# wangsibovictor/fora

Hardware: AMD Instinct MI355X
Metric: SSPPR queries/sec at eps=0.5 (higher is better)
Workload: dtype u64 fixed-point 2^-62 (f64 at the boundary)

## Files before the change

### fora_amd/csrc/fora_hip.hip

```cpp
#include "fora_kernels.h"
#include "fora_team.h"
#include "fora_bwd.h"
#include "fora_sweep.h"
#include "fora_tables.h"
#include "../../include/fora_hip.h"

#include <algorithm>
#include <cmath>
#include <cstdio>
#include <cstdlib>
#include <cstring>
#include <string>
#include <unordered_map>
#include <utility>
#include <vector>

using namespace fora;

namespace {

enum EvKind { EV_PUSH_POP, EV_PUSH_EXPAND, EV_WALK_ALLOC, EV_WALK, EV_OTHER, EV_BATCH, EV_PUSH_ACCUM, EV_WALK_ACCUM, EV_ROUND_SWEEP,
              EV_PUSH_TAIL, EV_PUSH_TEAM, EV_BWD, EV_COMBINE, EV_SP_COMPACT, EV_SEED_COMBINE,
              EV_SW_COMPACT, EV_SW_SORT, EV_SW_CUT };
struct EvPair { hipEvent_t a, b; EvKind kind; };
// ... 1415 lines not shown
                               (const int32_t *)c->g.d_col.get(), (const int32_t *)w.d_ids.get(), (unsigned long long *)w.d_cut.get(), hcap);
        }
        hipLaunchKernelGGL(k_sweep_scan, dim3(nr), dim3(BLOCK), 0, c->stream, d_rd, (uint32_t)r0, w.d_cut.get(), w.d_vol.get(), hcap, (uint64_t)c->g.nnz, w.d_out.get());
        if (maxL)
            hipLaunchKernelGGL(k_sweep_scatter<false>, dim3(gx(maxL), nr), dim3(BLOCK), 0, c->stream, d_rd, (uint32_t)r0, w.d_rank.get(), n, (const int32_t *)w.d_tids.get(), tcap,
                               (const uint32_t *)nullptr, (int32_t *)nullptr, (uint64_t *)nullptr, (uint64_t *)nullptr, (uint64_t)0);
    }
    ev.end();
    HIPCHK(c, hipMemcpyAsync(w.h_out.get(), w.d_out.get(), (size_t)nb * sizeof(SweepRowOut), hipMemcpyDeviceToHost, c->stream));
    HIPCHK(c, hipStreamSynchronize(c->stream));
    const hipError_t e = hipGetLastError();
    if (e != hipSuccess) return fail(c, FORA_E_HIP, std::string("sweep: ") + hipGetErrorString(e));
    w.rank_dirty = false;
    for (int i = 0; i < nb; i++) {
        const SweepRowOut &o = w.h_out.get()[i];
        sw.rows[(size_t)at[i]] = sweep_row_of(o.len, o.best, o.cut, o.vol, o.den);
        sw.edges += o.edges;
    }
    return FORA_OK;
}

int sweep_finish(fora_ctx *c, SweepRun &sw, const int32_t *sources, int nq, int64_t *row_ptr, fora_sweep_row *rows, fora_sweep_stats *out) {
    SweepResult &w = c->swp;
    sweep_skip_dangling(sw, sources, nq);
    sw.row_ptr[(size_t)nq] = (int64_t)sw.cur;
    if (int rc = sweep_reserve(c, sw.cur, sw.cur, (uint64_t)nq, (uint64_t)nq)) return rc;
    DevBuf<int64_t> at; DevBuf<int32_t> src;
    const size_t nd = sw.dang_at.size();
    if (nd) {
        HIPCHK(c, at.alloc(nd));
        HIPCHK(c, src.alloc(nd));
        HIPCHK(c, hipMemcpyAsync(at.get(), sw.dang_at.data(), nd * 8, hipMemcpyHostToDevice, c->stream));
        HIPCHK(c, hipMemcpyAsync(src.get(), sw.dang_src.data(), nd * 4, hipMemcpyHostToDevice, c->stream));
        hipLaunchKernelGGL(k_sweep_single, dim3((unsigned)((nd + BLOCK - 1) / BLOCK)), dim3(BLOCK), 0, c->stream, (uint32_t)nd, (const int64_t *)at.get(),
                           (const int32_t *)src.get(), w.d_ids.get(), w.d_cut.get(), w.d_vol.get(), (uint64_t)w.d_ids.size());
    }
    HIPCHK(c, hipStreamSynchronize(c->stream));
    const hipError_t e = hipGetLastError();
    if (e != hipSuccess) return fail(c, FORA_E_HIP, std::string("sweep result: ") + hipGetErrorString(e));
    ev_collect(c);
    w.entries = sw.cur;
    w.valid = true;
    memcpy(row_ptr, sw.row_ptr.data(), ((size_t)nq + 1) * 8);
    if (rows && nq) memcpy(rows, sw.rows.data(), (size_t)nq * sizeof(fora_sweep_row));
    if (out) {
        memset(out, 0, sizeof(*out));
        out->entries = sw.entries_len; out->max_row = sw.max_row; out->thr_fix = sw.thr; out->edges = sw.edges;
        out->batches = sw.batches; out->global_rows = sw.global_rows;
        out->compact_ms = c->tm.sw_compact_ms; out->sort_ms = c->tm.sw_sort_ms; out->cut_ms = c->tm.sw_cut_ms;
    }
    return FORA_OK;
}

void launch_walks(fora_ctx *c, const Dev &d, int nq, bool with_idx, uint32_t round, int nzh) {
    const WsPlan &p = c->ws.plan;
    const dim3 wg(walk_grid_x(c, nq), nq);
    const dim3 wgs(p.binned ? p.sub : 1u, nq);
    EvSpan ev(c, EV_WALK);
    if (with_idx) {
        if (!p.binned) hipLaunchKernelGGL(k_walk_idx<1>, wg, dim3(BLOCK), 0, c->stream, d);
        else if (!d.wide) hipLaunchKernelGGL(k_walk_idx<MAX_BINS>, wgs, dim3(BLOCK), 0, c->stream, d);
        else
            for (int lo = 0; lo < p.nbins; lo += p.pbins) {
                Dev dp = d;
                dp.bin_lo = lo;
                dp.bin_cnt = std::min(p.pbins, p.nbins - lo);
                const dim3 wgi = (dp.slot_major & 4u) ? dim3(wgs.y, wgs.x) : wgs;
                if (p.pbins > MAX_BINS_WIDE) hipLaunchKernelGGL(k_walk_idx<MAX_BINS_HUGE>, wgi, dim3(BIN_THREADS_HUGE), 0, c->stream, dp);
                else hipLaunchKernelGGL(k_walk_idx<MAX_BINS_WIDE>, wgi, dim3(BIN_THREADS_WIDE), 0, c->stream, dp);
                { const unsigned gx = acc_grid(c, dp, nq); hipLaunchKernelGGL((k_accum<true, true>), (dp.slot_major & 2u) ? dim3(nq, gx) : dim3(gx, nq), dim3(ACC_THREADS_WIDE), 0, c->stream, dp, 0); }
            }
    }
    const bool dg = p.binned && !d.wide && d.dg.colp && c->opt_.walk_dg != 0;
    const bool xl = dg && c->opt_.walk_dg != 1 && d.dg.invb;
    if (xl && with_idx) {
        ev.begin(EV_WALK_ACCUM);
        hipLaunchKernelGGL((k_accum<true, false>), dim3(p.nbins, nq), dim3(ACC_THREADS), 0, c->stream, d, 0);
        ev.begin(EV_WALK);
    }
    Dev dw = d;
    if (xl) { dw.nbins = (int32_t)d.dg.nbx; dw.acc_xl = d.dg.invb; }
    if (dg) {
        const size_t lds = (xl ? (size_t)((d.dg.H + 1) & ~1u) * 8 : 0) + (size_t)4 * d.dg.nrec * 4 + (((size_t)d.dg.nblk + 3) & ~(size_t)3);
#define FORA_DG_LAUNCH(NZH, B32, XLF) hipLaunchKernelGGL((k_walk_dg<NZH, B32, XLF>), wgs, dim3(DG_THREADS), lds, c->stream, dw, round)
        const int sel = (nzh ? 4 : 0) | (d.dg.bits32 ? 2 : 0) | (xl ? 1 : 0);
        switch (sel) {
        case 0: FORA_DG_LAUNCH(false, false, false); break;
        case 1: FORA_DG_LAUNCH(false, false, true); break;
        case 2: FORA_DG_LAUNCH(false, true, false); break;
        case 3: FORA_DG_LAUNCH(false, true, true); break;
        case 4: FORA_DG_LAUNCH(true, false, false); break;
        case 5: FORA_DG_LAUNCH(true, false, true); break;
        case 6: FORA_DG_LAUNCH(true, true, false); break;
        default: FORA_DG_LAUNCH(true, true, true); break;
        }
#undef FORA_DG_LAUNCH
    } else
        hipLaunchKernelGGL(k_walk_online<WALK_TO_PPR>, p.binned && !d.wide ? wgs : wg, dim3(BLOCK), 0, c->stream, d, round, nzh, (int32_t *)nullptr);
    ev.end();
    if (p.binned && !d.wide) {
        ev.begin(EV_WALK_ACCUM);
        hipLaunchKernelGGL((k_accum<true, false>), dim3(dw.nbins, nq), dim3(ACC_THREADS), 0, c->stream, dw, 0);
    }
}

static hipError_t ensure_active(Workspace &w) { return w.d_active.ensure((size_t)w.B); }
int push_balanced(fora_ctx *c, const int32_t *sources, int nq, bool with_idx) {
    HIPCHK(c, ensure_active(c->ws));
    const uint32_t chunks = slab_grid_x(c, std::min(nq, c->ws.B));
    Dev d = make_dev(c, nq, with_idx);
    EvSpan ev(c, EV_OTHER);
    hipLaunchKernelGGL(k_init_batch, dim3((nq + BLOCK - 1) / BLOCK), dim3(BLOCK), 0, c->stream, d, 1);
    ev.end();
    std::vector<uint8_t> active((size_t)nq, 1);
    std::vector<uint64_t> rsum_fix((size_t)nq, FIX_ONE), pops((size_t)nq, 0), relax((size_t)nq, 0);
    c->bal.h_rmax_used.assign((size_t)nq, c->par.rmax);
    c->bal.h_rounds.assign((size_t)nq, 1);
    for (int i = 0; i < nq; i++)
        if (is_dangling(c, sources[i])) active[i] = 0;
    for (int i = 0; i < nq; i++) if (active[i]) c->bal.h_rounds[i] = 0;
    double rmax = c->par.rmax * c->bal.start;
    for (int round = 0;; round++) {
        bool any = false;
        for (int i = 0; i < nq; i++) {
            if (!active[i]) continue;
            const double t = (!with_idx || rmax >= c->par.rmax) ? c->bal.t_walk : c->bal.t_idx;
            const double est = c->par.omega * std::ldexp((double)rsum_fix[i], -62) * (1 - c->par.alpha) * t;
            const double used = (double)pops[i] * c->bal.c_pop + (double)relax[i] * c->bal.c_edge;
            if (!(est > used)) active[i] = 0;
            else { any = true; c->bal.h_rmax_used[i] = rmax; c->bal.h_rounds[i] = round + 1; }
        }
        if (!any) break;
        if (round >= 64) return fail(c, FORA_E_OVERFLOW, "--balanced: rmax halved 64 times");
        HIPCHK(c, hipMemcpyAsync(c->ws.d_active.get(), active.data(), (size_t)nq, hipMemcpyHostToDevice, c->stream));
        if (round) {
            HIPCHK(c, c->ws.d_counters.zero(c->stream));
            int rc = reset_binned_counters(c);
            if (rc) return rc;
        }
        Dev dr = make_dev(c, nq, with_idx, rmax, c->par.omega);
        ev.begin(EV_OTHER);
        hipLaunchKernelGGL(k_topk_frontier, dim3(chunks, nq), dim3(BLOCK), 0, c->stream, dr, (const uint8_t *)c->ws.d_active.get());
        ev.end();
        int rc = run_push_levels(c, dr, nullptr, 0, true);
        if (rc) return rc;
        HIPCHK(c, hipMemcpy(c->h_qs.data(), c->ws.d_qs.get(), (size_t)nq * sizeof(QState), hipMemcpyDeviceToHost));
        for (int i = 0; i < nq; i++) {
            rsum_fix[i] = FIX_ONE - c->h_qs[i].reserved;
            pops[i] = c->h_qs[i].pops;
// ... 645 lines not shown
    if (!(alpha > 0 && alpha < 1) || !(rmax > 0) || !(omega >= 0)) return fail(c, FORA_E_ARG, "bad params");
    c->par.alpha = alpha; c->par.rmax = rmax; c->par.omega = omega; c->par.opt = opt ? 1 : 0; c->par.seed = seed;
    c->par.have = true;
    return FORA_OK;
}

int fora_hip_get_params(fora_ctx *c, double *rmax, double *omega) {
    if (!c || !c->par.have) return FORA_E_ARG;
    if (rmax) *rmax = c->par.rmax;
    if (omega) *omega = c->par.omega;
    return FORA_OK;
}

int fora_hip_set_batch(fora_ctx *c, int batch) {
    if (!c || batch < 0) return FORA_E_ARG;
    if (batch != c->batch_req) { (void)hipSetDevice(c->device); free_workspace(c); }
    c->batch_req = batch;
    return FORA_OK;
}
int fora_hip_get_batch(fora_ctx *c) { return c ? c->ws.B : FORA_E_ARG; }

int fora_hip_set_option(fora_ctx *c, const char *name, int64_t value) {
    if (!c || !name) return FORA_E_ARG;
    if (!strcmp(name, "reset")) {
        (void)hipSetDevice(c->device);
        free_workspace(c);
        c->opt_ = tunables_from_env();
        c->team_run.suspend = 0;
        apply_options(c);
        return FORA_OK;
    }
    if (!TEST_PATHS && schedule_option(name) && value != (strcmp(name, "rounds") ? (strcmp(name, "round_div") ? 0 : 4) : 1))
        return fail(c, FORA_E_ARG, std::string("option ") + name + ": the schedule experiments are not compiled into this library (build with -DFORA_TEST_PATHS=1: libfora_hip_test.so)");
    for (const auto &o : OPTIONS)
        if (!strcmp(name, o.name)) {
            if (c->opt_.*(o.field) == value) return FORA_OK;
            c->opt_.*(o.field) = value;
            if (o.layout) { (void)hipSetDevice(c->device); free_workspace(c); }
            apply_options(c);
            return FORA_OK;
        }
    return fail(c, FORA_E_ARG, std::string("unknown option ") + name);
}

int fora_hip_get_option(fora_ctx *c, const char *name, int64_t *value) {
    if (!name || !value) return FORA_E_ARG;
    if (!strcmp(name, "test_paths")) { *value = TEST_PATHS ? 1 : 0; return FORA_OK; }
    if (!strcmp(name, "diag_build")) { *value = FORA_DIAG_BUILD; return FORA_OK; }
    if (!c) return FORA_E_ARG;
    if (!strcmp(name, "bucket_retries")) { *value = (int64_t)c->retry.retries; return FORA_OK; }
    if (!strcmp(name, "team_fallbacks")) { *value = (int64_t)c->team_run.fallbacks; return FORA_OK; }
    if (!strcmp(name, "team_suspended")) { *value = c->team_run.suspend; return FORA_OK; }
    if (!strcmp(name, "team_members")) { *value = c->g.team.T; return FORA_OK; }
    if (!strcmp(name, "team_cooperative")) { *value = c->team_run.coop_ok && !c->team_run.coop_failed ? 1 : 0; return FORA_OK; }
    for (const auto &o : OPTIONS)
        if (!strcmp(name, o.name)) { *value = c->opt_.*(o.field); return FORA_OK; }
    return fail(c, FORA_E_ARG, std::string("unknown option ") + name);
}

int fora_hip_set_balanced(fora_ctx *c, int on, double start_scale, double c_pop, double c_edge, double t_walk, double t_idx) {
    if (!c) return FORA_E_ARG;
    const Balanced def;
    c->bal.on = on != 0;
    c->bal.start = start_scale > 0 ? start_scale : def.start;
    c->bal.c_pop = c_pop > 0 ? c_pop : def.c_pop;
    c->bal.c_edge = c_edge > 0 ? c_edge : def.c_edge;
    c->bal.t_walk = t_walk > 0 ? t_walk : def.t_walk;
    c->bal.t_idx = t_idx > 0 ? t_idx : def.t_idx;
    return FORA_OK;
}

static uint64_t host_index_sizes(const fora_ctx *c, uint64_t *off, uint64_t *cnt) {
    uint64_t total = 0;
    for (int32_t v = 0; v < c->g.n; v++) {
        const size_t deg = (size_t)(c->g.h_row_ptr[v + 1] - c->g.h_row_ptr[v]);
        unsigned long num_rw;
        if (c->par.opt) num_rw = (unsigned long)ceil(deg * c->par.rmax * (1 - c->par.alpha) * c->par.omega);
        else num_rw = (unsigned long)ceil(deg * c->par.rmax * c->par.omega);
        if (off) off[v] = total;
        if (cnt) cnt[v] = num_rw;
        total += num_rw;
    }
    return total;
}

int fora_hip_index_sizes(fora_ctx *c, uint64_t *total, uint64_t *off, uint64_t *cnt) {
    if (!c || !c->g.n || !c->par.have) return fail(c, FORA_E_ARG, "set_graph and set_params first");
    const uint64_t t = host_index_sizes(c, off, cnt);
    if (total) *total = t;
    return FORA_OK;
}

int fora_hip_build_index(fora_ctx *c) {
    if (!c || !c->g.n || !c->par.have) return fail(c, FORA_E_ARG, "set_graph and set_params first");
    HIPCHK(c, hipSetDevice(c->device));
    std::vector<uint64_t> off((size_t)c->g.n), cnt((size_t)c->g.n);
    const uint64_t total = host_index_sizes(c, off.data(), cnt.data());
    free_index(c);
    Index ix;
    HIPCHK(c, ix.d_rw_idx.alloc(std::max<uint64_t>(1, total)));
    HIPCHK(c, ix.d_idx_off.alloc((size_t)c->g.n));
    HIPCHK(c, ix.d_idx_cnt.alloc((size_t)c->g.n));
    HIPCHK(c, hipMemcpy(ix.d_idx_off.get(), off.data(), (size_t)c->g.n * 8, hipMemcpyHostToDevice));
    HIPCHK(c, hipMemcpy(ix.d_idx_cnt.get(), cnt.data(), (size_t)c->g.n * 8, hipMemcpyHostToDevice));
    ix.len = total;
    c->retry.div = 1;
// ... 1106 lines not shown
```

### fora_amd/csrc/fora_kernels.h

```cpp
#pragma once
#include <hip/hip_runtime.h>
#include <stdint.h>
#include <type_traits>
#include "fora_consts.h"
#include "fora_diag.h"

namespace fora {

constexpr int BLOCK = 256;
constexpr uint32_t PUSH_SEG = 256;
constexpr uint32_t WALK_SEG = 1024;
#ifndef FORA_TEST_PATHS
#define FORA_TEST_PATHS 0
#endif
constexpr bool TEST_PATHS = FORA_TEST_PATHS != 0;
constexpr uint64_t FIX_ONE = 1ull << 62;
constexpr int MAX_LEVELS = 1 << 15;
#ifndef FORA_ACC_THREADS
#define FORA_ACC_THREADS 512
#endif
constexpr int ACC_THREADS = FORA_ACC_THREADS;
#ifndef FORA_ACC_THREADS_WIDE
#define FORA_ACC_THREADS_WIDE 1024
#endif
// ... 1981 lines not shown
                    WalkItem w = {};
                    w.j0 = (uint64_t)k * WALK_SEG;
                    const uint64_t left = num - w.j0;
                    w.cnt = left < WALK_SEG ? (uint32_t)left : WALK_SEG;
                    w.idx_pos = ioff + w.j0;
                    w.v = v;
                    d.wit[sb + off + k] = wit_pack(w);
                }
            }
        }
    }
}

enum { WALK_TO_PPR = 0, WALK_TO_INDEX = 1 };

__device__ __forceinline__ int32_t walk_one(const Dev &d, uint32_t start, uint64_t j, uint32_t stream,
                                            uint32_t round, int nzh, uint32_t &steps) {
    int64_t beg; uint64_t deg;
    node_row(d, start, beg, deg);
    if (deg == 0) return (int32_t)start;
    uint32_t cur = start;
    uint32_t w[4];
    for (uint32_t t = 0;; t++) {
        if ((t & 1u) == 0)
            philox4x32_10(start, (uint32_t)j,
                          (uint32_t)((j >> 32) & 0xFFFFu) | ((round & 0xFFu) << 16) | (((t >> 1) & 0xFFu) << 24),
                          stream ^ ((t >> 9) * 0x9E3779B9u), d.seed_lo, d.seed_hi, w);
        const uint32_t ws = (t & 1u) ? w[2] : w[0], wm = (t & 1u) ? w[3] : w[1];
        if (!(nzh && t == 0) && ws < d.alpha32) return (int32_t)cur;
        if (t) node_row(d, cur, beg, deg);
        if (deg > 0)
            cur = (uint32_t)d.col[beg + (int64_t)(((uint64_t)wm * deg) >> 32)];
        else
            cur = start;
        steps++;
    }
}

#ifndef FORA_STAGE
#define FORA_STAGE 320
#endif
#ifndef FORA_WALK_WPE
#define FORA_WALK_WPE 6
#endif
constexpr int STAGE = FORA_STAGE;
struct WaveStage {
    uint64_t *pk;
    uint32_t *bcnt;
    uint32_t *bbase;
    uint32_t *fill;
    uint32_t count;
    const uint32_t *xl;
};
template <int ST, bool XLD = false>
__device__ __forceinline__ void stage_flush(const Dev &d, int q, WaveStage &st) {
    const int lane = threadIdx.x & 63;
    const uint64_t slab = (uint64_t)q * d.n;
    const uint64_t bk0 = SubBuckets::first_of(d.pbins, d.sub, d.bk_cap, q, blockIdx.x), bstride = SubBuckets::stride_of(d.sub, d.bk_cap);
    st.bcnt[lane] = 0;
    st.bcnt[lane + 64] = 0;
    __builtin_amdgcn_wave_barrier();
    constexpr uint64_t NONE = ~0ull;
    uint32_t rk[ST / 64];
    uint64_t wv[ST / 64];
#pragma unroll
    for (int k = 0; k < ST / 64; k++) {
        const uint32_t m = k * 64 + lane;
        wv[k] = NONE;
        if (m < st.count) {
            wv[k] = st.pk[m];
            if (XLD) {
                const uint32_t lo = (uint32_t)wv[k], u = lo & ((1u << WPACK_SHIFT) - 1), blk = u >> 6;
                const uint32_t qd = __umulhi(blk, d.dg.nbx_magic);
                const uint32_t dest = ((blk - qd * d.dg.nbx) << BIN_SHIFT) | (qd << 6) | (u & 63u);
                wv[k] = (wv[k] & 0xFFFFFFFF00000000ull) | ((lo & ~((1u << WPACK_SHIFT) - 1)) | dest);
            }
            rk[k] = atomicAdd(&st.bcnt[((uint32_t)wv[k] & ((1u << WPACK_SHIFT) - 1)) >> BIN_SHIFT], 1u);
        }
    }
    __builtin_amdgcn_wave_barrier();
    {
        const uint32_t c0 = lane < d.nbins ? st.bcnt[lane] : 0, c1 = lane + 64 < d.nbins ? st.bcnt[lane + 64] : 0;
        uint32_t t0, t1;
        const uint32_t o0 = wave_excl_scan(c0, t0), o1 = wave_excl_scan(c1, t1);
        if (c0) st.bbase[lane] = atomicAdd(&st.fill[lane], c0);
        if (c1) st.bbase[lane + 64] = atomicAdd(&st.fill[lane + 64], c1);
        st.bcnt[lane] = o0;
        st.bcnt[lane + 64] = t0 + o1;
    }
    __builtin_amdgcn_wave_barrier();
#pragma unroll
    for (int k = 0; k < ST / 64; k++)
        if (wv[k] != NONE) st.pk[st.bcnt[((uint32_t)wv[k] & ((1u << WPACK_SHIFT) - 1)) >> BIN_SHIFT] + rk[k]] = wv[k];
    __builtin_amdgcn_wave_barrier();
#pragma unroll
    for (int k = 0; k < ST / 64; k++) {
        const uint32_t m = k * 64 + lane;
        if (m < st.count) {
            const uint64_t pk = st.pk[m];
            const uint32_t dd = (uint32_t)pk & ((1u << WPACK_SHIFT) - 1);
            const uint32_t b = dd >> BIN_SHIFT;
            const uint32_t pos = st.bbase[b] + (m - st.bcnt[b]);
            if (pos < d.bk_cap) __builtin_nontemporal_store(pk, &d.bk_inc[bk0 + (uint64_t)b * bstride + pos]);
            else atomicAdd((unsigned long long *)&d.ppr[slab + (st.xl ? st.xl[dd] : dd)], (unsigned long long)(pk >> WPACK_SHIFT));
        }
    }
    __builtin_amdgcn_wave_barrier();
    st.count = 0;
}
template <int ST, bool XLD = false, bool CHECKW = true>
__device__ __forceinline__ void stage_emit(const Dev &d, int q, WaveStage &st, bool has, uint32_t dest, uint64_t w) {
    if (CHECKW && has && w >= WPACK_MAXW) {
        atomicAdd((unsigned long long *)&d.ppr[(uint64_t)q * d.n + (st.xl ? st.xl[dest] : dest)], (unsigned long long)w);
        has = false;
    }
    const unsigned long long mask = __ballot(has);
    if (!mask) return;
    if (has) {
        const uint32_t pos = st.count + sp_mbcnt(mask);
        st.pk[pos] = (uint64_t)dest | (w << WPACK_SHIFT);
    }
    st.count += (uint32_t)__popcll(mask);
    if (st.count > ST - 64) stage_flush<ST, XLD>(d, q, st);
}
#define WAVE_STAGE_DECL_N(st, NWAVES, ST)                                                           \
    __shared__ uint64_t st##_pk[NWAVES][ST];                                                        \
    __shared__ uint32_t st##_bcnt[NWAVES][MAX_BINS], st##_bbase[NWAVES][MAX_BINS];                 \
    __shared__ uint32_t st##_fill[MAX_BINS];                                                        \
    WaveStage st;                                                                                   \
    st.pk = st##_pk[threadIdx.x >> 6];                                                              \
    st.bcnt = st##_bcnt[threadIdx.x >> 6]; st.bbase = st##_bbase[threadIdx.x >> 6];                 \
    st.fill = st##_fill; st.count = 0; st.xl = nullptr;
#define WAVE_STAGE_DECL(st) WAVE_STAGE_DECL_N(st, BLOCK / 64, STAGE)

template <int NB>
__global__ void __launch_bounds__(BinThreads<NB>::value) k_walk_idx(Dev d) {
    constexpr int NT = BinThreads<NB>::value;
    constexpr int EPT = NB > MAX_BINS ? FORA_IDX_EPT_WIDE : BIN_EPT;
    constexpr uint32_t CHUNK = NT * EPT;
    constexpr uint32_t PAD = NB > MAX_BINS ? FORA_RUN_PAD_WIDE : 1;
    constexpr bool BINNED = NB > 1;
    constexpr bool WIDE = NB > MAX_BINS;
    constexpr int BS = WIDE ? BIN_SHIFT_WIDE : BIN_SHIFT;
    constexpr uint32_t BSZ = 1u << BS;
    constexpr int IB = NT == 256 ? 8 : NT == 512 ? 9 : 10;
    constexpr int DB = WIDE ? BS : WPACK_SHIFT;
    static_assert(DB + IB + 1 <= 32, "stage word: destination | item | carries-one-more-unit");
    __shared__ uint64_t s_j0[NT], s_pos[NT], s_incr[NT], s_rem[NT];
    __shared__ uint32_t s_pref[NT + 1], s_w[NT / 64];
    __shared__ uint32_t s_cnt[NB], s_lofs[NB + 1], s_fill[NB];
    __shared__ uint32_t s_msg[BINNED ? CHUNK : 1];
    __shared__ uint16_t s_bin[BINNED ? CHUNK : 1];
    const bool slot_major = NB > MAX_BINS && (d.slot_major & 4u);
    const int q = slot_major ? blockIdx.x : blockIdx.y;
    const uint32_t bx = slot_major ? blockIdx.y : blockIdx.x, gx = slot_major ? gridDim.y : gridDim.x;
    const uint32_t nitems = (uint32_t)min((uint64_t)d.wit_count[q * CSTRIDE], d.wit_cap);
    if (!nitems || *d.err) return;
    const WalkItemP *items = d.wit + (uint64_t)q * d.wit_cap;
    const uint64_t slab = (uint64_t)q * d.n;
    const uint32_t bin_lo = (uint32_t)d.bin_lo;
    const BinExchange<NB, NT, PAD> ex{s_cnt, s_lofs, s_fill, s_w, SubBuckets(d.bk_count, d.pbins, d.sub, d.bk_cap, q, bx), (uint32_t)d.bin_cnt};
    if (BINNED) ex.load_fills();
    constexpr uint32_t GRAN = FORA_TILE_GRAN_WALK;
    const uint32_t ntiles = (nitems + NT - 1) / NT;
    const uint32_t seg_len = ntiles * GRAN;
    for (uint32_t tile = bx; tile < ntiles; tile += gx) {
        const uint32_t i = tile_pos<GRAN>(threadIdx.x, tile, seg_len);
        uint32_t cnt = 0;
        if (i < nitems) {
            const WalkItem w = wit_load(&items[i]);
            s_j0[threadIdx.x] = w.j0; s_pos[threadIdx.x] = w.idx_pos;
            s_incr[threadIdx.x] = w.incr; s_rem[threadIdx.x] = w.rem;
            cnt = w.idx_n;
        }
        uint32_t total;
        const uint32_t pre = block_excl_scan_n<NT>(cnt, s_w, total);
        s_pref[threadIdx.x] = pre;
        if (threadIdx.x == 0) s_pref[NT] = total;
        __syncthreads();
        for (uint32_t cb = 0; cb < total; cb += CHUNK) {
            uint32_t dest[EPT], rank[EPT], li[EPT];
            const uint32_t e0 = cb + threadIdx.x * EPT;
            uint32_t lo = e0 < total ? pref_find<NT>(s_pref, e0) : 0;
#pragma unroll
// ... 134 lines not shown
                        if (deg0 == 0) done = (int32_t)start;
                        else active = true;
                    }
                    const uint32_t want = (uint32_t)__popcll(idle);
                    wptr += want < avail ? want : avail;
                    while (wptr < wend && s_pref[cur_item + 1] <= wptr) cur_item++;
                }
                if (active)
                    philox4x32_10(start, (uint32_t)wj,
                                  (uint32_t)((wj >> 32) & 0xFFFFu) | ((round & 0xFFu) << 16) | (((t >> 1) & 0xFFu) << 24),
                                  stream ^ ((t >> 9) * 0x9E3779B9u), d.seed_lo, d.seed_hi, rw);
            }
            if (active) {
                const uint32_t ws = (it & 1u) ? rw[2] : rw[0], wm = (it & 1u) ? rw[3] : rw[1];
                if (!(nzh && t == 0) && ws < d.alpha32) {
                    done = (int32_t)cur;
                    active = false;
                } else {
                    if (t) cur = walk_move(d, cur, start, wm);
                    else if (d.rp32) cur = colp_at(d, (uint64_t)beg0 + (((uint64_t)wm * deg0) >> 32));
                    else cur = (uint32_t)d.col[beg0 + (int64_t)(((uint64_t)wm * deg0) >> 32)];
                    t++;
                    steps++;
                }
            }
            if (staged) {
                stage_emit<STAGE>(d, q, st, done >= 0, (uint32_t)done, wgt);
            } else if (done >= 0) {
                if (MODE == WALK_TO_INDEX) idx_out[opos] = done;
                else atomicAdd((unsigned long long *)&d.ppr[slab + (uint32_t)done], (unsigned long long)wgt);
            }
        }
        __syncthreads();
    }
    if (staged && st.count) stage_flush<STAGE>(d, q, st);
    if (staged) {
        __syncthreads();
        for (uint32_t i = threadIdx.x; i < (uint32_t)d.nbins; i += BLOCK) bkc[(uint64_t)i * d.sub] = st.fill[i];
    }
    const uint64_t ws = wave_sum((uint64_t)steps);
    __syncthreads();
    if ((threadIdx.x & 63) == 0) s_w[threadIdx.x >> 6] = (uint32_t)ws;
    __syncthreads();
    if (threadIdx.x == 0) {
        const unsigned long long bs = (unsigned long long)s_w[0] + s_w[1] + s_w[2] + s_w[3];
        if (bs) atomicAdd(d.tot_steps, bs);
    }
}

#ifndef FORA_DG_THREADS
#define FORA_DG_THREADS 512
#endif
#ifndef FORA_DG_STAGE
#define FORA_DG_STAGE 256
#endif
#ifndef FORA_DG_WPE
#define FORA_DG_WPE 6
#endif
constexpr int DG_THREADS = FORA_DG_THREADS;
constexpr int DG_STAGE = FORA_DG_STAGE;
#ifndef FORA_DG_TILE
#define FORA_DG_TILE 256
#endif
constexpr int DG_TILE = FORA_DG_TILE;
typedef uint32_t __attribute__((aligned(1))) u32_unaligned;
template <bool BITS32>
__device__ __forceinline__ uint32_t dg_colp_at(const WalkDG &g, uint32_t e) {
    if (BITS32) {
        const uint32_t at = g.bits * e;
        const uint32_t w = *(const u32_unaligned *)((const char *)g.colp + (at >> 3));
        return (w >> (at & 7)) & ((1u << g.bits) - 1u);
    }
    uint32_t word, sh;
    if (BITS32) { const uint32_t at = g.bits * e; word = at >> 5; sh = at & 31; }
    else { const uint64_t at = (uint64_t)g.bits * e; word = (uint32_t)(at >> 5); sh = (uint32_t)at & 31; }
    const U32Pair cw = *(const U32Pair *)(g.colp + word);
    const uint64_t both = ((uint64_t)cw.b << 32) | cw.a;
    return (uint32_t)(both >> sh) & ((1u << g.bits) - 1u);
}
template <bool NZH, bool BITS32, bool XL>
__global__ void __launch_bounds__(DG_THREADS) __attribute__((amdgpu_waves_per_eu(FORA_DG_WPE, 8))) k_walk_dg(Dev d, uint32_t round) {
    constexpr int NW = DG_THREADS / 64;
    extern __shared__ __attribute__((aligned(16))) uint64_t dg_lds64[];
    constexpr int WT = DG_TILE / NW;
    static_assert(WT >= 1 && WT <= 64, "a lane loads one item of its wave's tile");
    struct __attribute__((aligned(16))) TileItem { uint64_t jb, rem, incr; uint32_t v, vp; };
    static_assert(sizeof(TileItem) == 32, "two uint4");
    __shared__ TileItem w_item[NW][WT];
    __shared__ uint32_t w_pref[NW][WT + 1], s_w[NW];
    __shared__ unsigned long long w_self[XL ? NW : 1][XL ? WT : 1];
    __shared__ uint32_t s_ticket;
    const int q = blockIdx.y;
    const uint32_t nitems = (uint32_t)min((uint64_t)d.wit_count[q * CSTRIDE], d.wit_cap);
    if (!nitems || *d.err) return;
    const WalkDG &g = d.dg;
    const uint32_t H = g.H, ts = g.ts;
    unsigned long long *s_hub = (unsigned long long *)dg_lds64;
    uint32_t *dg_lds = (uint32_t *)(dg_lds64 + (XL ? ((H + 1) & ~1u) : 0));
    uint4 *s_rec = (uint4 *)dg_lds;
    const uint32_t ncls = g.nrec - H;
    const uint8_t *s_T = (const uint8_t *)(dg_lds + 4 * g.nrec);
    for (uint32_t i = threadIdx.x; i < g.nrec; i += DG_THREADS) s_rec[i < H ? ncls + i : i - H] = make_uint4(g.rec[i], g.rec[g.nrec + i], g.rec[2 * g.nrec + i], 0u);
    for (uint32_t i = threadIdx.x; i < (g.nblk + 3) / 4; i += DG_THREADS) dg_lds[4 * g.nrec + i] = ((const uint32_t *)g.T)[i];
    if (XL) for (uint32_t i = threadIdx.x; i < H; i += DG_THREADS) s_hub[i] = 0;
    const WalkItemP *items = d.wit + (uint64_t)q * d.wit_cap;
    const uint64_t slab = (uint64_t)q * d.n;
    const uint32_t stream = (uint32_t)d.src[q];
    const int lane = threadIdx.x & 63, wid = __builtin_amdgcn_readfirstlane((int)(threadIdx.x >> 6));
    uint32_t steps = 0;
    WAVE_STAGE_DECL_N(st, NW, DG_STAGE)
    if (XL) st.xl = g.invb;
    uint32_t *bkc = d.bk_count + (uint64_t)q * d.pbins * d.sub + blockIdx.x;
    for (uint32_t i = threadIdx.x; i < (uint32_t)MAX_BINS; i += DG_THREADS) st.fill[i] = i < (uint32_t)d.nbins ? bkc[(uint64_t)i * d.sub] : 0;
    if (threadIdx.x == 0) s_ticket = 0;
    __syncthreads();
    auto move = [&](uint32_t cur, uint32_t startp, uint32_t wm) -> uint32_t {
        uint32_t r = ncls + cur;
        if (cur >= H) r = s_T[(cur - H) >> ts];
        const uint4 rc = s_rec[r];
        const uint32_t dg = rc.y;
        const uint32_t e = rc.z + (cur - rc.x) * dg + __umulhi(wm, dg);
        const uint32_t nx = dg_colp_at<BITS32>(g, e);
        return dg ? nx : startp;
    };
    bool pend = false;
    uint32_t pend_node = 0;
    uint64_t pend_w = 0;
    unsigned long long *s_self = w_self[XL ? wid : 0];
    TileItem *s_item = w_item[wid];
    uint32_t *s_pref = w_pref[wid];
    if (XL && lane < WT) s_self[lane] = 0;
    uint32_t gen = 0, tag = 0;
    auto flush_self = [&]() {
        if (!XL) return;
        const unsigned long long sv = lane < WT ? s_self[lane] : 0ull;
        const uint32_t dn = lane < WT ? s_item[lane].vp : 0u;
        if (lane < WT && sv) s_self[lane] = 0;
        if (sv && dn < H) atomicAdd(&s_hub[dn], sv);
        bool has = sv != 0 && dn >= H;
        if (has && sv >= WPACK_MAXW) {
            atomicAdd((unsigned long long *)&d.ppr[slab + g.inv[dn]], sv);
            has = false;
        }
        stage_emit<DG_STAGE, true, false>(d, q, st, has, dn - H, (uint64_t)sv);
    };
    const uint32_t ntiles = (nitems + WT - 1) / WT;
    const uint32_t tstride = gridDim.x * NW;
    bool more = true;
    auto take_tile = [&]() -> uint32_t {
        uint32_t k = 0;
        if (lane == 0) k = atomicAdd(&s_ticket, 1u);
        return dg_ticket_tile(blockIdx.x, (uint32_t)NW, tstride, (uint32_t)__builtin_amdgcn_readfirstlane((int)k));
    };
    uint32_t wptr = 0, wend = 0;
    uint32_t cur_item = 0;
    bool big = false;
    auto advance = [&]() {
        while (wptr < wend && (uint32_t)__builtin_amdgcn_readfirstlane((int)s_pref[cur_item + 1]) <= wptr) cur_item++;
    };
    bool active = false;
    uint32_t cur = 0, start = 0, startp = 0, c1 = 0, c2 = 0, c3 = 0;
    const uint32_t c2_round = (round & 0xFFu) << 16;
    uint64_t wgt = 0;
    for (;;) {
        bool fin = false;
        const unsigned long long idle = __ballot(!active);
        if (idle && wptr == wend) {
            while (wptr == wend && more) {
                const uint32_t tile = take_tile();
                if (tile >= ntiles) { more = false; break; }
                if (gen) flush_self();
                gen++;
                const uint32_t i = tile * WT + lane;
                const bool have = lane < WT && i < nitems;
                WalkItem w = {};
                if (have) {
                    const uint64_t *wp = (const uint64_t *)&items[i];
                    const uint64_t x0 = NT_LOAD(wp), x1 = NT_LOAD(wp + 1), x3 = NT_LOAD(wp + 3);
                    w = wit_unpack(x0, x1, 0, x3);
                }
                const uint32_t cnt = have ? w.cnt - w.idx_n : 0u;
                uint32_t total;
                const uint32_t pre = wave_excl_scan(cnt, total);
                if (have) {
                    TileItem it;
                    it.jb = w.j0 + w.idx_n - pre;
                    it.rem = w.rem; it.incr = w.incr;
                    it.v = w.v; it.vp = g.perm[w.v];
                    s_item[lane] = it;
                }
                if (__ballot(have && w.incr + 1 >= WPACK_MAXW)) big = true;
                if (lane < WT) s_pref[lane] = pre;
                if (lane == 0) s_pref[WT] = total;
                __builtin_amdgcn_fence(__ATOMIC_RELEASE, "wavefront");
                __builtin_amdgcn_wave_barrier();
                wptr = 0; wend = total; cur_item = 0;
                advance();
            }
        }
        const uint32_t avail = wend - wptr;
        if (!avail && idle == ~0ull) break;
        if (avail && idle) {
            const uint32_t rank = sp_mbcnt(idle);
            if (!active && rank < avail) {
                const uint32_t e = wptr + rank;
                uint32_t item = cur_item;
                while (s_pref[item + 1] <= e) item++;
                const uint4 ia = ((const uint4 *)&s_item[item])[0], ib = ((const uint4 *)&s_item[item])[1];
                const uint64_t wj = (((uint64_t)ia.y << 32) | ia.x) + e;
                const uint64_t rem = ((uint64_t)ia.w << 32) | ia.z;
                wgt = (((uint64_t)ib.y << 32) | ib.x) + (wj < rem ? 1 : 0);
                start = ib.z;
                startp = ib.w;
                c1 = (uint32_t)wj;
                c2 = ((uint32_t)(wj >> 32) & 0xFFFFu) | c2_round;
                c3 = stream;
                cur = startp;
                tag = (gen << 6) | item;
                fin = startp >= g.zero_first;
                active = !fin;
            }
            const uint32_t want = (uint32_t)__popcll(idle);
            wptr += want < avail ? want : avail;
            advance();
            __builtin_amdgcn_wave_barrier();
        }
        if (active) {
            uint32_t rw[4];
            philox4x32_10(start, c1, c2, c3, d.seed_lo, d.seed_hi, rw);
            const uint32_t later = (c2 >> 24) | (c3 ^ stream);
            c2 += 1u << 24;
            if (__ballot(c2 < (1u << 24))) {
                asm volatile("" ::: "memory");
                if (c2 < (1u << 24)) c3 = stream ^ ((c3 ^ stream) + 0x9E3779B9u);
            }
            if (!(NZH && later == 0) && rw[0] < d.alpha32) {
                fin = true;
            } else {
                cur = move(diag::dg_from(cur, later), startp, rw[1]);
                steps++;
                if (rw[2] < d.alpha32) {
                    fin = true;
                } else {
                    cur = move(diag::dg_from(cur, 1u), startp, rw[3]);
                    steps++;
                }
            }
            active = !fin;
        }
        if (XL) {
            const bool self = fin && cur == startp && tag >= (gen << 6);
            if (self) atomicAdd(&s_self[tag & 63u], (unsigned long long)wgt);
            const bool away = fin && !self;
            if (away && cur < H) atomicAdd(&s_hub[cur], (unsigned long long)wgt);
            const bool over = big && wgt >= WPACK_MAXW;
            if (away && cur >= H && over) atomicAdd((unsigned long long *)&d.ppr[slab + g.inv[cur]], (unsigned long long)wgt);
            stage_emit<DG_STAGE, true, false>(d, q, st, away && cur >= H && !over, cur - H, wgt);
        } else {
            stage_emit<DG_STAGE>(d, q, st, pend, pend_node, pend_w);
            pend = fin;
            if (pend) { pend_node = g.inv[cur]; pend_w = wgt; }
        }
    }
    if (!XL) stage_emit<DG_STAGE>(d, q, st, pend, pend_node, pend_w);
    if (gen) flush_self();
    if (st.count) stage_flush<DG_STAGE, XL>(d, q, st);
    __syncthreads();
    for (uint32_t i = threadIdx.x; i < (uint32_t)d.nbins; i += DG_THREADS) bkc[(uint64_t)i * d.sub] = st.fill[i];
    if (XL) for (uint32_t i = threadIdx.x; i < H; i += DG_THREADS) {
        const unsigned long long hv = s_hub[i];
        if (hv) atomicAdd((unsigned long long *)&d.ppr[slab + g.inv[i]], hv);
    }
    const uint64_t ws = wave_sum((uint64_t)steps);
    if (lane == 0) s_w[wid] = (uint32_t)ws;
    __syncthreads();
    if (threadIdx.x == 0) {
        unsigned long long bs = 0;
#pragma unroll
        for (int w = 0; w < NW; w++) bs += s_w[w];
        if (bs) atomicAdd(d.tot_steps, bs);
    }
}

__global__ void __launch_bounds__(BLOCK) k_ppr_sum(Dev d) {
    const int q = blockIdx.y;
    const uint64_t slab = (uint64_t)q * d.n;
    uint64_t acc = 0;
    const uint64_t step = (uint64_t)gridDim.x * BLOCK;
    for (uint64_t v0 = (uint64_t)blockIdx.x * BLOCK + threadIdx.x; v0 < (uint64_t)d.n; v0 += step * SLAB_UNROLL) {
        uint64_t x[SLAB_UNROLL];
        slab_load(x, d.ppr, slab, v0, step, (uint64_t)d.n);
#pragma unroll
        for (int u = 0; u < SLAB_UNROLL; u++) acc += x[u];
    }
    acc = wave_sum(acc);
    if ((threadIdx.x & 63) == 0 && acc) atomicAdd(&d.qs[q].ppr_sum, (unsigned long long)acc);
}

__global__ void __launch_bounds__(BLOCK) k_walk_counts_f64(int32_t n, const double *residue, double rsum,
                                                           double omega, double alpha, int opt,
                                                           uint64_t *num_s_rw, uint64_t *n_rw) {
    double check_rsum = rsum;
    if (opt) check_rsum *= (1 - alpha);
    const uint64_t N = check_rsum == 0.0 ? 0 : (uint64_t)(omega * check_rsum);
    const int v = blockIdx.x * BLOCK + threadIdx.x;
    if (v == 0) *n_rw = N;
    if (v >= n) return;
    double r = residue[v];
    uint64_t num = 0;
    if (r > 0 && check_rsum != 0.0) {
        if (opt) r = r * (1 - alpha);
        num = walk_count(r, check_rsum, N);
    }
    num_s_rw[v] = num;
}

__global__ void __launch_bounds__(BLOCK) k_walks_raw(Dev d, uint32_t stream, uint32_t round, int nzh,
                                                     const int32_t *starts, const uint64_t *js, int64_t count,
                                                     int32_t *dests) {
// ... 285 lines not shown
```

### fora_amd/csrc/fora_tables.h

```cpp
#pragma once
#include "fora_consts.h"

#include <algorithm>
#include <cstddef>
#include <vector>

namespace fora {


inline std::vector<uint32_t> in_degrees(size_t n, const int32_t *col, size_t nnz) {
    std::vector<uint32_t> indeg(n, 0);
    for (size_t e = 0; e < nnz; e++) indeg[(size_t)col[e]]++;
    return indeg;
}
inline std::vector<uint32_t> top_by_indegree(const std::vector<uint32_t> &indeg, size_t H) {
    std::vector<uint32_t> order(indeg.size());
    for (size_t v = 0; v < order.size(); v++) order[v] = (uint32_t)v;
    H = std::min(H, order.size());
    std::partial_sort(order.begin(), order.begin() + (ptrdiff_t)H, order.end(),
                      [&](uint32_t a, uint32_t b) { return indeg[a] != indeg[b] ? indeg[a] > indeg[b] : a < b; });
    order.resize(H);
    return order;
}
template <class F> std::vector<uint32_t> pack_bits(uint64_t count, uint32_t bits, F value_of) {
    std::vector<uint32_t> pk((size_t)((count * bits + 31) / 32) + 2, 0);
    for (uint64_t e = 0; e < count; e++) {
        const uint64_t at = e * bits;
        const uint64_t x = (uint64_t)(uint32_t)value_of(e) << (at & 31);
        pk[at >> 5] |= (uint32_t)x;
        pk[(at >> 5) + 1] |= (uint32_t)(x >> 32);
    }
    return pk;
}


struct RowBasics {
    bool ok = true;
    std::vector<uint64_t> rowinfo;
    std::vector<uint32_t> deg;
    int64_t n_dangling = 0;
};
inline RowBasics make_row_basics(int32_t n, const int64_t *row_ptr) {
    RowBasics r;
    r.rowinfo.resize((size_t)n);
    r.deg.resize((size_t)n);
    for (int32_t v = 0; v < n; v++) {
        const uint64_t dg = (uint64_t)(row_ptr[v + 1] - row_ptr[v]);
        r.n_dangling += dg == 0;
        if (dg > 0xFFFFFFFFull) { r.ok = false; return r; }
        r.deg[(size_t)v] = (uint32_t)dg;
        r.rowinfo[(size_t)v] = ((uint64_t)row_ptr[v] << 24) | std::min<uint64_t>(dg, DEG_SAT);
    }
    return r;
}


struct CompactWalk {
    uint32_t bits = 0;
    std::vector<uint32_t> rp32, colp;
};
inline CompactWalk make_compact_walk(int32_t n, const int64_t *row_ptr, const int32_t *col) {
    CompactWalk w;
    w.bits = 1;
    while ((1ull << w.bits) < (uint64_t)n) w.bits++;
    if (w.bits > 31) w.bits = 31;
    w.rp32.resize((size_t)n + 1);
    for (int32_t v = 0; v <= n; v++) w.rp32[(size_t)v] = (uint32_t)row_ptr[v];
    w.colp = pack_bits((uint64_t)row_ptr[n], w.bits, [&](uint64_t e) { return col[e]; });
    return w;
}


constexpr size_t WALK_DG_LDS_CAP = 28 * 1024;
struct DgTables {
    bool have = false;
    uint32_t H = 0, nrec = 0, ts = 0, bits = 0, zero_first = 0, bits32 = 0;
    uint32_t np = 0;
    std::vector<uint32_t> perm, inv, rec, colp;
    std::vector<uint8_t> T;
    uint32_t nbx = 0, nbx_magic = 0;
    std::vector<uint32_t> invb;
};
inline DgTables make_walk_dg(int32_t n, const int64_t *row_ptr, const int32_t *col, int64_t dg_hubs) {
    DgTables t;
    const uint64_t nnz = (uint64_t)row_ptr[n];
    std::vector<uint32_t> order((size_t)n);
    for (int32_t v = 0; v < n; v++) order[(size_t)v] = (uint32_t)v;
    auto degree = [&](uint32_t v) { return (uint32_t)(row_ptr[v + 1] - row_ptr[v]); };
    std::stable_sort(order.begin(), order.end(), [&](uint32_t a, uint32_t b) { return degree(a) > degree(b); });
    uint32_t H = 0, K = 0;
    for (uint32_t h : {256u, 512u, 1024u, 2048u, 4096u}) {
        if (dg_hubs > 0 && (int64_t)h < dg_hubs) continue;
        const uint32_t hh = std::min<uint32_t>(h, (uint32_t)n);
        uint32_t k = 0;
        for (size_t i = hh; i < (size_t)n; i++) if (i == hh || degree(order[i]) != degree(order[i - 1])) k++;
        if (k <= 255) { H = hh; K = k; break; }
    }
    if (H == 0 && !(n <= 256)) return DgTables{};
    if (n <= 256) { H = (uint32_t)n; K = 0; }
    uint32_t ts = 6;
    while ((((uint64_t)n + 256ull * (1ull << ts)) >> ts) > 8192) ts++;
    const uint32_t blk = 1u << ts;
    const uint32_t nrec = H + K;
    t.rec.assign((size_t)3 * nrec, 0);
    t.perm.resize((size_t)n);
    uint32_t *first = t.rec.data(), *rdeg = t.rec.data() + nrec, *base = t.rec.data() + 2 * (size_t)nrec;
    uint64_t edge = 0;
    uint32_t id = 0, zero_first = 0xFFFFFFFFu;
    for (uint32_t i = 0; i < H; i++) {
        const uint32_t v = order[i];
        t.perm[v] = id; first[i] = id; rdeg[i] = degree(v); base[i] = (uint32_t)edge;
        if (rdeg[i] == 0 && zero_first == 0xFFFFFFFFu) zero_first = id;
        edge += rdeg[i]; id++;
    }
    uint32_t k = 0;
    for (size_t i = H; i < (size_t)n;) {
        size_t j = i;
        const uint32_t dg = degree(order[i]);
        while (j < (size_t)n && degree(order[j]) == dg) j++;
        const uint32_t r = H + k;
        first[r] = id; rdeg[r] = dg; base[r] = (uint32_t)edge;
        if (dg == 0 && zero_first == 0xFFFFFFFFu) zero_first = id;
        for (size_t u = i; u < j; u++) t.perm[order[u]] = id + (uint32_t)(u - i);
        const uint32_t cnt = (uint32_t)(j - i), padded = (cnt + blk - 1) / blk * blk;
        for (uint32_t b = 0; b < padded / blk; b++) t.T.push_back((uint8_t)k);
        edge += (uint64_t)cnt * dg;
// ... 185 lines not shown
```

Measured before the change: 7058.

## Shrink walk_dg LDS footprint: drop bbase array, 16-bit prefixes, retune stage/tile

The degree-grouped walk kernel now uses a staging variant that folds each bin's global base minus its local offset into the per-wave bcnt array, so the separate bbase shared array is no longer needed. Tile prefix sums are stored as 16-bit values, guarded by a static_assert. The stage size goes from 256 to 384 and the tile size from 256 to 128. A host-side query option reports the kernel's workgroups per CU, and the kernel selection and LDS size computation are moved into helper functions. The aim is to trade LDS between staging capacity and occupancy, and a larger stage risks lowering occupancy.

```diff
diff --git a/fora_amd/csrc/fora_hip.hip b/fora_amd/csrc/fora_hip.hip
--- a/fora_amd/csrc/fora_hip.hip
+++ b/fora_amd/csrc/fora_hip.hip
@@ -1491,6 +1491,21 @@
     return FORA_OK;
 }
 
+typedef void (*WalkDgKernel)(Dev, uint32_t);
+static WalkDgKernel walk_dg_kernel(bool nzh, bool bits32, bool xl) {
+    switch ((nzh ? 4 : 0) | (bits32 ? 2 : 0) | (xl ? 1 : 0)) {
+    case 0: return k_walk_dg<false, false, false>;
+    case 1: return k_walk_dg<false, false, true>;
+    case 2: return k_walk_dg<false, true, false>;
+    case 3: return k_walk_dg<false, true, true>;
+    case 4: return k_walk_dg<true, false, false>;
+    case 5: return k_walk_dg<true, false, true>;
+    case 6: return k_walk_dg<true, true, false>;
+    default: return k_walk_dg<true, true, true>;
+    }
+}
+static size_t walk_dg_lds(const WalkDG &g, bool xl) { return walk_dg_lds_bytes(g.H, g.nrec, g.nblk, xl); }
+
 void launch_walks(fora_ctx *c, const Dev &d, int nq, bool with_idx, uint32_t round, int nzh) {
     const WsPlan &p = c->ws.plan;
     const dim3 wg(walk_grid_x(c, nq), nq);
@@ -1520,20 +1535,7 @@
     Dev dw = d;
     if (xl) { dw.nbins = (int32_t)d.dg.nbx; dw.acc_xl = d.dg.invb; }
     if (dg) {
-        const size_t lds = (xl ? (size_t)((d.dg.H + 1) & ~1u) * 8 : 0) + (size_t)4 * d.dg.nrec * 4 + (((size_t)d.dg.nblk + 3) & ~(size_t)3);
-#define FORA_DG_LAUNCH(NZH, B32, XLF) hipLaunchKernelGGL((k_walk_dg<NZH, B32, XLF>), wgs, dim3(DG_THREADS), lds, c->stream, dw, round)
-        const int sel = (nzh ? 4 : 0) | (d.dg.bits32 ? 2 : 0) | (xl ? 1 : 0);
-        switch (sel) {
-        case 0: FORA_DG_LAUNCH(false, false, false); break;
-        case 1: FORA_DG_LAUNCH(false, false, true); break;
-        case 2: FORA_DG_LAUNCH(false, true, false); break;
-        case 3: FORA_DG_LAUNCH(false, true, true); break;
-        case 4: FORA_DG_LAUNCH(true, false, false); break;
-        case 5: FORA_DG_LAUNCH(true, false, true); break;
-        case 6: FORA_DG_LAUNCH(true, true, false); break;
-        default: FORA_DG_LAUNCH(true, true, true); break;
-        }
-#undef FORA_DG_LAUNCH
+        hipLaunchKernelGGL(walk_dg_kernel(nzh != 0, d.dg.bits32 != 0, xl), wgs, dim3(DG_THREADS), walk_dg_lds(d.dg, xl), c->stream, dw, round);
     } else
         hipLaunchKernelGGL(k_walk_online<WALK_TO_PPR>, p.binned && !d.wide ? wgs : wg, dim3(BLOCK), 0, c->stream, d, round, nzh, (int32_t *)nullptr);
     ev.end();
@@ -2285,6 +2287,18 @@
     if (!strcmp(name, "team_fallbacks")) { *value = (int64_t)c->team_run.fallbacks; return FORA_OK; }
     if (!strcmp(name, "team_suspended")) { *value = c->team_run.suspend; return FORA_OK; }
     if (!strcmp(name, "team_members")) { *value = c->g.team.T; return FORA_OK; }
+    if (!strcmp(name, "walk_dg_wgs_per_cu")) {
+        const WalkDG &g = c->g.walk.dg;
+        int wgs = 0;
+        if (g.colp) {
+            const bool xl = c->opt_.walk_dg != 1 && g.invb;
+            (void)hipSetDevice(c->device);
+            if (hipOccupancyMaxActiveBlocksPerMultiprocessor(&wgs, (const void *)walk_dg_kernel(false, g.bits32 != 0, xl), DG_THREADS, walk_dg_lds(g, xl)) != hipSuccess)
+                return fail(c, FORA_E_HIP, "hipOccupancyMaxActiveBlocksPerMultiprocessor(k_walk_dg)");
+        }
+        *value = wgs;
+        return FORA_OK;
+    }
     if (!strcmp(name, "team_cooperative")) { *value = c->team_run.coop_ok && !c->team_run.coop_failed ? 1 : 0; return FORA_OK; }
     for (const auto &o : OPTIONS)
         if (!strcmp(name, o.name)) { *value = c->opt_.*(o.field); return FORA_OK; }
diff --git a/fora_amd/csrc/fora_kernels.h b/fora_amd/csrc/fora_kernels.h
--- a/fora_amd/csrc/fora_kernels.h
+++ b/fora_amd/csrc/fora_kernels.h
@@ -2057,7 +2057,7 @@
     uint32_t count;
     const uint32_t *xl;
 };
-template <int ST, bool XLD = false>
+template <int ST, bool XLD = false, bool ONE = false>
 __device__ __forceinline__ void stage_flush(const Dev &d, int q, WaveStage &st) {
     const int lane = threadIdx.x & 63;
     const uint64_t slab = (uint64_t)q * d.n;
@@ -2068,6 +2068,7 @@
     constexpr uint64_t NONE = ~0ull;
     uint32_t rk[ST / 64];
     uint64_t wv[ST / 64];
+    uint32_t dl0 = 0, dl1 = 0;
 #pragma unroll
     for (int k = 0; k < ST / 64; k++) {
         const uint32_t m = k * 64 + lane;
@@ -2088,8 +2089,13 @@
         const uint32_t c0 = lane < d.nbins ? st.bcnt[lane] : 0, c1 = lane + 64 < d.nbins ? st.bcnt[lane + 64] : 0;
         uint32_t t0, t1;
         const uint32_t o0 = wave_excl_scan(c0, t0), o1 = wave_excl_scan(c1, t1);
-        if (c0) st.bbase[lane] = atomicAdd(&st.fill[lane], c0);
-        if (c1) st.bbase[lane + 64] = atomicAdd(&st.fill[lane + 64], c1);
+        if (ONE) {
+            if (c0) dl0 = atomicAdd(&st.fill[lane], c0) - o0;
+            if (c1) dl1 = atomicAdd(&st.fill[lane + 64], c1) - (t0 + o1);
+        } else {
+            if (c0) st.bbase[lane] = atomicAdd(&st.fill[lane], c0);
+            if (c1) st.bbase[lane + 64] = atomicAdd(&st.fill[lane + 64], c1);
+        }
         st.bcnt[lane] = o0;
         st.bcnt[lane + 64] = t0 + o1;
     }
@@ -2098,6 +2104,11 @@
     for (int k = 0; k < ST / 64; k++)
         if (wv[k] != NONE) st.pk[st.bcnt[((uint32_t)wv[k] & ((1u << WPACK_SHIFT) - 1)) >> BIN_SHIFT] + rk[k]] = wv[k];
     __builtin_amdgcn_wave_barrier();
+    if (ONE) {
+        st.bcnt[lane] = dl0;
+        st.bcnt[lane + 64] = dl1;
+        __builtin_amdgcn_wave_barrier();
+    }
 #pragma unroll
     for (int k = 0; k < ST / 64; k++) {
         const uint32_t m = k * 64 + lane;
@@ -2105,7 +2116,7 @@
             const uint64_t pk = st.pk[m];
             const uint32_t dd = (uint32_t)pk & ((1u << WPACK_SHIFT) - 1);
             const uint32_t b = dd >> BIN_SHIFT;
-            const uint32_t pos = st.bbase[b] + (m - st.bcnt[b]);
+            const uint32_t pos = ONE ? st.bcnt[b] + m : st.bbase[b] + (m - st.bcnt[b]);
             if (pos < d.bk_cap) __builtin_nontemporal_store(pk, &d.bk_inc[bk0 + (uint64_t)b * bstride + pos]);
             else atomicAdd((unsigned long long *)&d.ppr[slab + (st.xl ? st.xl[dd] : dd)], (unsigned long long)(pk >> WPACK_SHIFT));
         }
@@ -2113,7 +2124,7 @@
     __builtin_amdgcn_wave_barrier();
     st.count = 0;
 }
-template <int ST, bool XLD = false, bool CHECKW = true>
+template <int ST, bool XLD = false, bool CHECKW = true, bool ONE = false>
 __device__ __forceinline__ void stage_emit(const Dev &d, int q, WaveStage &st, bool has, uint32_t dest, uint64_t w) {
     if (CHECKW && has && w >= WPACK_MAXW) {
         atomicAdd((unsigned long long *)&d.ppr[(uint64_t)q * d.n + (st.xl ? st.xl[dest] : dest)], (unsigned long long)w);
@@ -2126,7 +2137,7 @@
         st.pk[pos] = (uint64_t)dest | (w << WPACK_SHIFT);
     }
     st.count += (uint32_t)__popcll(mask);
-    if (st.count > ST - 64) stage_flush<ST, XLD>(d, q, st);
+    if (st.count > ST - 64) stage_flush<ST, XLD, ONE>(d, q, st);
 }
 #define WAVE_STAGE_DECL_N(st, NWAVES, ST)                                                           \
     __shared__ uint64_t st##_pk[NWAVES][ST];                                                        \
@@ -2135,6 +2146,14 @@
     WaveStage st;                                                                                   \
     st.pk = st##_pk[threadIdx.x >> 6];                                                              \
     st.bcnt = st##_bcnt[threadIdx.x >> 6]; st.bbase = st##_bbase[threadIdx.x >> 6];                 \
+    st.fill = st##_fill; st.count = 0; st.xl = nullptr;
+#define WAVE_STAGE_DECL_ONE(st, NWAVES, ST)                                                         \
+    __shared__ uint64_t st##_pk[NWAVES][ST];                                                        \
+    __shared__ uint32_t st##_bcnt[NWAVES][MAX_BINS];                                                \
+    __shared__ uint32_t st##_fill[MAX_BINS];                                                        \
+    WaveStage st;                                                                                   \
+    st.pk = st##_pk[threadIdx.x >> 6];                                                              \
+    st.bcnt = st##_bcnt[threadIdx.x >> 6]; st.bbase = nullptr;                                      \
     st.fill = st##_fill; st.count = 0; st.xl = nullptr;
 #define WAVE_STAGE_DECL(st) WAVE_STAGE_DECL_N(st, BLOCK / 64, STAGE)
 
@@ -2375,7 +2394,7 @@
 #define FORA_DG_THREADS 512
 #endif
 #ifndef FORA_DG_STAGE
-#define FORA_DG_STAGE 256
+#define FORA_DG_STAGE 384
 #endif
 #ifndef FORA_DG_WPE
 #define FORA_DG_WPE 6
@@ -2383,7 +2402,7 @@
 constexpr int DG_THREADS = FORA_DG_THREADS;
 constexpr int DG_STAGE = FORA_DG_STAGE;
 #ifndef FORA_DG_TILE
-#define FORA_DG_TILE 256
+#define FORA_DG_TILE 128
 #endif
 constexpr int DG_TILE = FORA_DG_TILE;
 typedef uint32_t __attribute__((aligned(1))) u32_unaligned;
@@ -2410,7 +2429,9 @@
     struct __attribute__((aligned(16))) TileItem { uint64_t jb, rem, incr; uint32_t v, vp; };
     static_assert(sizeof(TileItem) == 32, "two uint4");
     __shared__ TileItem w_item[NW][WT];
-    __shared__ uint32_t w_pref[NW][WT + 1], s_w[NW];
+    static_assert((uint64_t)WT * WALK_SEG <= 0xFFFFu, "a tile's walk count fits the 16-bit prefix sums");
+    __shared__ uint16_t w_pref[NW][WT + 1];
+    __shared__ uint32_t s_w[NW];
     __shared__ unsigned long long w_self[XL ? NW : 1][XL ? WT : 1];
     __shared__ uint32_t s_ticket;
     const int q = blockIdx.y;
@@ -2431,7 +2452,7 @@
     const uint32_t stream = (uint32_t)d.src[q];
     const int lane = threadIdx.x & 63, wid = __builtin_amdgcn_readfirstlane((int)(threadIdx.x >> 6));
     uint32_t steps = 0;
-    WAVE_STAGE_DECL_N(st, NW, DG_STAGE)
+    WAVE_STAGE_DECL_ONE(st, NW, DG_STAGE)
     if (XL) st.xl = g.invb;
     uint32_t *bkc = d.bk_count + (uint64_t)q * d.pbins * d.sub + blockIdx.x;
     for (uint32_t i = threadIdx.x; i < (uint32_t)MAX_BINS; i += DG_THREADS) st.fill[i] = i < (uint32_t)d.nbins ? bkc[(uint64_t)i * d.sub] : 0;
@@ -2451,7 +2472,7 @@
     uint64_t pend_w = 0;
     unsigned long long *s_self = w_self[XL ? wid : 0];
     TileItem *s_item = w_item[wid];
-    uint32_t *s_pref = w_pref[wid];
+    uint16_t *s_pref = w_pref[wid];
     if (XL && lane < WT) s_self[lane] = 0;
     uint32_t gen = 0, tag = 0;
     auto flush_self = [&]() {
@@ -2465,7 +2486,7 @@
             atomicAdd((unsigned long long *)&d.ppr[slab + g.inv[dn]], sv);
             has = false;
         }
-        stage_emit<DG_STAGE, true, false>(d, q, st, has, dn - H, (uint64_t)sv);
+        stage_emit<DG_STAGE, true, false, true>(d, q, st, has, dn - H, (uint64_t)sv);
     };
     const uint32_t ntiles = (nitems + WT - 1) / WT;
     const uint32_t tstride = gridDim.x * NW;
@@ -2513,8 +2534,8 @@
                     s_item[lane] = it;
                 }
                 if (__ballot(have && w.incr + 1 >= WPACK_MAXW)) big = true;
-                if (lane < WT) s_pref[lane] = pre;
-                if (lane == 0) s_pref[WT] = total;
+                if (lane < WT) s_pref[lane] = (uint16_t)pre;
+                if (lane == 0) s_pref[WT] = (uint16_t)total;
                 __builtin_amdgcn_fence(__ATOMIC_RELEASE, "wavefront");
                 __builtin_amdgcn_wave_barrier();
                 wptr = 0; wend = total; cur_item = 0;
@@ -2578,16 +2599,16 @@
             if (away && cur < H) atomicAdd(&s_hub[cur], (unsigned long long)wgt);
             const bool over = big && wgt >= WPACK_MAXW;
             if (away && cur >= H && over) atomicAdd((unsigned long long *)&d.ppr[slab + g.inv[cur]], (unsigned long long)wgt);
-            stage_emit<DG_STAGE, true, false>(d, q, st, away && cur >= H && !over, cur - H, wgt);
+            stage_emit<DG_STAGE, true, false, true>(d, q, st, away && cur >= H && !over, cur - H, wgt);
         } else {
-            stage_emit<DG_STAGE>(d, q, st, pend, pend_node, pend_w);
+            stage_emit<DG_STAGE, false, true, true>(d, q, st, pend, pend_node, pend_w);
             pend = fin;
             if (pend) { pend_node = g.inv[cur]; pend_w = wgt; }
         }
     }
-    if (!XL) stage_emit<DG_STAGE>(d, q, st, pend, pend_node, pend_w);
+    if (!XL) stage_emit<DG_STAGE, false, true, true>(d, q, st, pend, pend_node, pend_w);
     if (gen) flush_self();
-    if (st.count) stage_flush<DG_STAGE, XL>(d, q, st);
+    if (st.count) stage_flush<DG_STAGE, XL, true>(d, q, st);
     __syncthreads();
     for (uint32_t i = threadIdx.x; i < (uint32_t)d.nbins; i += DG_THREADS) bkc[(uint64_t)i * d.sub] = st.fill[i];
     if (XL) for (uint32_t i = threadIdx.x; i < H; i += DG_THREADS) {
diff --git a/fora_amd/csrc/fora_tables.h b/fora_amd/csrc/fora_tables.h
--- a/fora_amd/csrc/fora_tables.h
+++ b/fora_amd/csrc/fora_tables.h
@@ -72,6 +72,9 @@
 
 
 constexpr size_t WALK_DG_LDS_CAP = 28 * 1024;
+inline size_t walk_dg_lds_bytes(uint32_t H, uint32_t nrec, uint32_t nblk, bool xl) {
+    return (xl ? (size_t)((H + 1) & ~1u) * 8 : 0) + (size_t)4 * nrec * 4 + (((size_t)nblk + 3) & ~(size_t)3);
+}
 struct DgTables {
     bool have = false;
     uint32_t H = 0, nrec = 0, ts = 0, bits = 0, zero_first = 0, bits32 = 0;
```

Result: faster. 7143, median of 6 (+1.2%).
